# UDC-GAC/pRIblast

Measured on AMD Instinct MI355X. Metric: query RNAs/sec in `ris` step, higher is better.
Workload: dtype f64

## Files before the change

### priblast_amd/csrc/gapped_lds.hip

```cpp
#include <algorithm>
#include <type_traits>

#include "gapped_args.hpp"
#include "search_device.hpp"
#include "search_kernels.hpp"

namespace prb {

#ifdef PRB_GAP_PROFILE
constexpr int kProfSlots = 24;
__device__ unsigned long long g_gap_prof[10 * kProfSlots];
struct GapProf {
  unsigned long long last, acc[kProfSlots];
  int cells_now = 0, cells_prev = 0;
  __device__ __forceinline__ void start() {
    for (int i = 0; i < kProfSlots; i++) acc[i] = 0;
    last = __builtin_amdgcn_s_memtime();
  }
  __device__ __forceinline__ void mark(int r) {
    const unsigned long long t = __builtin_amdgcn_s_memtime();
    acc[r] += t - last;
    last = t;
  }
  __device__ __forceinline__ void count(int r) { acc[r] += 1; }
  __device__ __forceinline__ void flush(int kind) {
    if ((threadIdx.x & 63) == 0)
      for (int i = 0; i < kProfSlots; i++) atomicAdd(&g_gap_prof[kind * kProfSlots + i], acc[i]);
  }
};
#define GP_MARK(r) prof.mark(r)
#define GP_COUNT(r) prof.count(r)
#else
struct GapProf {
  __device__ __forceinline__ void start() {}
  __device__ __forceinline__ void flush(int) {}
};
#define GP_MARK(r)
#define GP_COUNT(r)
#endif

namespace {

constexpr int kInitStage = 16;
struct Tier0 {
#ifndef PRB_T0_CAPR
#define PRB_T0_CAPR 48
#define PRB_T0_WGCU 4
#endif
#ifndef PRB_T0_ACC_GLOBAL
#define PRB_T0_ACC_GLOBAL false
#endif
  static constexpr int kG = 8, kCapD = 32, kCapR = PRB_T0_CAPR, kGroups = 32, kWavesPerSimd = PRB_T0_WGCU, kWgPerCu = PRB_T0_WGCU;
  static constexpr bool kResumable = true;
  static constexpr bool kResumes = false;
  static constexpr bool kPairSteps = true;
  static constexpr bool kAccGlobal = PRB_T0_ACC_GLOBAL;
};
#ifndef PRB_T12_ACC_GLOBAL
#define PRB_T12_ACC_GLOBAL true
#endif
#ifndef PRB_T12_WPS
#define PRB_T12_WPS (PRB_T12_ACC_GLOBAL ? 4 : 3)
#endif
#ifndef PRB_T1_CAPD
#define PRB_T1_CAPD 40
#define PRB_T1_CAPR 64
#define PRB_T1_GROUPS 32
#define PRB_T1_WGCU (PRB_T12_ACC_GLOBAL ? 4 : 3)
#endif
struct Tier1 {
  static constexpr int kG = 8, kCapD = PRB_T1_CAPD, kCapR = PRB_T1_CAPR, kGroups = PRB_T1_GROUPS, kWavesPerSimd = PRB_T12_WPS, kWgPerCu = PRB_T1_WGCU;
  static constexpr bool kResumable = true, kResumes = true;
  using From = Tier0;
  using FromRec = Rec32;
  static constexpr bool kPairSteps = false;
  static constexpr bool kAccGlobal = PRB_T12_ACC_GLOBAL;
};
struct Tier2 {
  static constexpr int kG = 16, kCapD = 64, kCapR = 120, kGroups = 16, kWavesPerSimd = PRB_T12_WPS, kWgPerCu = PRB_T12_ACC_GLOBAL ? 4 : 3;
  static constexpr bool kResumable = true, kResumes = true;
  using From = Tier1;
  using FromRec = Rec32;
  static constexpr bool kPairSteps = false;
  static constexpr bool kAccGlobal = PRB_T12_ACC_GLOBAL;
};
struct Tier3 {
  static constexpr int kG = 64, kCapD = 128, kCapR = 512, kGroups = 1, kWavesPerSimd = 4, kWgPerCu = 16;
  static constexpr bool kResumable = false, kResumes = true;
  using From = Tier2;
  using FromRec = Rec32;
  static constexpr bool kPairSteps = false;
  static constexpr bool kAccGlobal = false;
};

struct Rec32W {
  using word = uint32_t;
  static constexpr bool kBases = false;
  static __device__ __forceinline__ word pack(int i, int j, int pred, int type, int, int) {
    return (word)i | ((word)j << 8) | ((word)pred << 16) | ((word)type << 25);
  }
  static __device__ __forceinline__ int i(word v) { return v & 0xFF; }
  static __device__ __forceinline__ int j(word v) { return (v >> 8) & 0xFF; }
  static __device__ __forceinline__ int pred(word v) { return (v >> 16) & 0x1FF; }
  static __device__ __forceinline__ int type(word v) { return (v >> 25) & 7; }
  static __device__ __forceinline__ int qa(word) { return 0; }
  static __device__ __forceinline__ int da(word) { return 0; }
};
struct Rec64 {
  using word = uint64_t;
  static constexpr bool kBases = true;
  static __device__ __forceinline__ word pack(int i, int j, int pred, int type, int qa, int da) {
    return (word)(uint32_t)i | ((word)(uint32_t)j << 16) | ((word)type << 32) | ((word)qa << 36) | ((word)da << 40) |
           ((word)(uint32_t)pred << 44);
  }
  static __device__ __forceinline__ int i(word v) { return (int)(v & 0xFFFF); }
  static __device__ __forceinline__ int j(word v) { return (int)((v >> 16) & 0xFFFF); }
  static __device__ __forceinline__ int pred(word v) { return (int)(v >> 44); }
  static __device__ __forceinline__ int type(word v) { return (int)((v >> 32) & 0xF); }
  static __device__ __forceinline__ int qa(word v) { return (int)((v >> 36) & 0xF); }
  static __device__ __forceinline__ int da(word v) { return (int)((v >> 40) & 0xF); }
};
static_assert(Tier3::kCapD + 16 <= 255 && Tier3::kCapR <= 512 && Tier0::kCapR * 8 >= 6 * kInitStage * 4 && Tier2::kCapD + 16 <= 127 && Tier2::kCapR <= 127, "Rec32 field widths");
static_assert(Tier0::kCapD <= Tier1::kCapD && Tier1::kCapD <= Tier2::kCapD && Tier2::kCapD <= Tier3::kCapD && Tier0::kCapR <= Tier1::kCapR &&
                  Tier1::kCapR <= Tier2::kCapR && Tier2::kCapR <= Tier3::kCapR,
              "a tier continues the dumps of the one before it");

template <class T, class Rec> struct LdsState {
  double eq[T::kCapD], ed[T::kCapD];
  double hyb[T::kCapR];
  typename Rec::word info[T::kCapR];
  static constexpr int kPtabLen = (T::kCapD + 7) & ~7;
  alignas(8) uint8_t ptab[3][kPtabLen];
  uint8_t qb[T::kCapD + 16], db[T::kCapD + 16];
};
template <class T, class Rec, bool kAccGlobal = T::kAccGlobal> struct LdsLive : LdsState<T, Rec> {};
template <class T, class Rec> struct LdsLive<T, Rec, true> {
  double hyb[T::kCapR];
  typename Rec::word info[T::kCapR];
  static constexpr int kPtabLen = (T::kCapD + 7) & ~7;
  alignas(8) uint8_t ptab[3][kPtabLen];
  uint8_t qb[T::kCapD + 16], db[T::kCapD + 16];
};
template <class T, class Rec> struct LdsStore {
  using R = Rec;
  static constexpr bool kResumable = T::kResumable;
  static constexpr bool kAccGlobal = T::kAccGlobal;
  static constexpr int kCapD = T::kCapD;
  LdsLive<T, Rec> &s;
  double *acc;
  __device__ __forceinline__ int cap_d() const { return T::kCapD; }
  __device__ __forceinline__ int cap_r() const { return T::kCapR; }
  __device__ __forceinline__ double &eq(int i) const {
    if constexpr (T::kAccGlobal) return acc[i];
    else return s.eq[i];
  }
  __device__ __forceinline__ double &ed(int i) const {
    if constexpr (T::kAccGlobal) return acc[T::kCapD + i];
    else return s.ed[i];
  }
  __device__ __forceinline__ double &hyb(int r) const { return s.hyb[r]; }
  __device__ __forceinline__ typename Rec::word &info(int r) const { return s.info[r]; }
  __device__ __forceinline__ uint8_t &ptab(int row, int i) const { return s.ptab[row][i]; }
  __device__ __forceinline__ int ptab_len() const { return LdsState<T, Rec>::kPtabLen; }
  __device__ __forceinline__ int win_len() const { return T::kCapD + 16; }
  __device__ __forceinline__ uint8_t &qb(int t) const { return s.qb[t]; }
  __device__ __forceinline__ uint8_t &db(int t) const { return s.db[t]; }
};
struct HbmStore {
  using R = Rec64;
  static constexpr bool kResumable = false;
  static constexpr bool kAccGlobal = false;
  double *eq_, *ed_, *hyb_;
  uint64_t *info_;
  uint8_t *ptab_, *qb_, *db_;
  int capd, capr;
  __device__ __forceinline__ int cap_d() const { return capd; }
  __device__ __forceinline__ int cap_r() const { return capr; }
  __device__ __forceinline__ double &eq(int i) const { return eq_[i]; }
  __device__ __forceinline__ double &ed(int i) const { return ed_[i]; }
  __device__ __forceinline__ double &hyb(int r) const { return hyb_[r]; }
  __device__ __forceinline__ uint64_t &info(int r) const { return info_[r]; }
  __device__ __forceinline__ uint8_t &ptab(int row, int i) const { return ptab_[(size_t)row * (capd + 4) + i]; }
  __device__ __forceinline__ int ptab_len() const { return capd + 4; }
  __device__ __forceinline__ int win_len() const { return capd + 16; }
  __device__ __forceinline__ uint8_t &qb(int t) const { return qb_[t]; }
  __device__ __forceinline__ uint8_t &db(int t) const { return db_[t]; }
};

template <bool kLds> __device__ __forceinline__ void group_sync() {
  if (kLds) {
    __builtin_amdgcn_fence(__ATOMIC_RELEASE, "wavefront");
    __builtin_amdgcn_wave_barrier();
    __builtin_amdgcn_fence(__ATOMIC_ACQUIRE, "wavefront");
  } else {
    __builtin_amdgcn_fence(__ATOMIC_RELEASE, "workgroup");
    __builtin_amdgcn_wave_barrier();
    __builtin_amdgcn_fence(__ATOMIC_ACQUIRE, "workgroup");
  }
}

template <class Store> __device__ __forceinline__ void acc_sync() {
  if constexpr (Store::kAccGlobal) {
    __builtin_amdgcn_fence(__ATOMIC_RELEASE, "workgroup");
    __builtin_amdgcn_wave_barrier();
    __builtin_amdgcn_fence(__ATOMIC_ACQUIRE, "workgroup");
  }
}

template <int kCtrl> __device__ __forceinline__ double dpp_f64(double x) {
  const int lo = __builtin_amdgcn_update_dpp(0, __double2loint(x), kCtrl, 0xF, 0xF, false);
  const int hi = __builtin_amdgcn_update_dpp(0, __double2hiint(x), kCtrl, 0xF, 0xF, false);
  return __hiloint2double(hi, lo);
}
template <int kCtrl> __device__ __forceinline__ int dpp_i32(int x) { return __builtin_amdgcn_update_dpp(0, x, kCtrl, 0xF, 0xF, false); }
__device__ __forceinline__ void group_min_halves(double &te, int &key, bool halves) {
  double m = te;
  m = __builtin_fmin(m, dpp_f64<0xB1>(m));
  m = __builtin_fmin(m, dpp_f64<0x4E>(m));
  const double m8 = __builtin_fmin(m, dpp_f64<0x141>(m));
  m = halves ? m : m8;
  int k = te == m ? key : 0x7fffffff;
  k = min(k, dpp_i32<0xB1>(k));
  k = min(k, dpp_i32<0x4E>(k));
  const int k8 = min(k, dpp_i32<0x141>(k));
  te = m;
  key = halves ? k : k8;
}
template <int G> __device__ __forceinline__ void group_min(double &te, int &key) {
  if (G == 8 || G == 16) {
    double m = te;
    m = __builtin_fmin(m, dpp_f64<0xB1>(m));
    m = __builtin_fmin(m, dpp_f64<0x4E>(m));
    m = __builtin_fmin(m, dpp_f64<0x141>(m));
    if (G == 16) m = __builtin_fmin(m, dpp_f64<0x140>(m));
    int k = te == m ? key : 0x7fffffff;
    k = min(k, dpp_i32<0xB1>(k));
    k = min(k, dpp_i32<0x4E>(k));
    k = min(k, dpp_i32<0x141>(k));
    if (G == 16) k = min(k, dpp_i32<0x140>(k));
    te = m;
    key = k;
  } else if (G == 64) {
    group_min<16>(te, key);
#pragma unroll
    for (int m = 16; m <= 32; m <<= 1) {
      const double ote = __shfl_xor(te, m);
      const int ok = __shfl_xor(key, m);
      if (ote < te || (ote == te && ok < key)) {
        te = ote;
        key = ok;
      }
    }
  } else {
#pragma unroll
    for (int m = G / 2; m >= 1; m >>= 1) {
      const double ote = __shfl_xor(te, m);
      const int ok = __shfl_xor(key, m);
      if (ote < te || (ote == te && ok < key)) {
        te = ote;
        key = ok;
      }
    }
  }
}

struct DirResult {
  bool overflow;
  int best;
};

struct SeqBases {
  const uint8_t *qenc;
  const float *qacc, *qcond, *dacc, *dcond;
};
struct HitCtx {
  int64_t x, out0;
  int64_t qo, dbase;
  HitState h;
  int query, id, qn;
  int diag_q, diag_d, diag_len, ndiag, nleft, nright;
  bool unsorted, ovf;
  bool resumed;
  int tier0;
};
struct DirState {
  double min_e;
  double acc_prev;
  int min_ci, min_cj;
  int length, best, nrec, lo, tq0, td0;
  int staged;
  int resume_i0, resume_dstart;
  bool overflow;
};

template <int G, bool kLds, class Store>
__device__ __forceinline__ void stage_acc(const SeqBases &sb, const HitCtx &c, int flag, int delta, const Store &S, int gl, DirState &d, int L0,
                                          int nb, float *scratch ) {
  const float *qacc = sb.qacc + c.qo, *qcond = sb.qcond + c.qo, *dacc = sb.dacc + c.dbase, *dcond = sb.dcond + c.dbase;
  const DirOrigin og = dir_origin(c.h, flag);
  auto term = [&](int k, int len) -> float {
    if (flag == 0) {
      const int p = og.q_start - len;
      return k == 0 ? qacc[p] : k == 1 ? qacc[p + 1] : k == 2 ? qcond[p + delta] : dcond[og.id_end + len];
    }
    const int p = og.id_start - len;
    return k == 0 ? qcond[og.q_start + len] : k == 3 ? dacc[p] : k == 4 ? dacc[p + 1] : dcond[p + delta];
  };
  if (scratch) {
    for (int t = gl; t < nb; t += G) {
      const int len = L0 + t;
      if (len < d.tq0) {
        scratch[0 * nb + t] = term(0, len);
        if (flag == 0) {
          scratch[1 * nb + t] = term(1, len);
          scratch[2 * nb + t] = term(2, len);
        }
      }
      if (len < d.td0) {
        scratch[3 * nb + t] = term(3, len);
        if (flag == 1) {
          scratch[4 * nb + t] = term(4, len);
          scratch[5 * nb + t] = term(5, len);
        }
      }
    }
    group_sync<kLds>();
  }
  auto get = [&](int k, int t) -> float { return scratch ? scratch[k * nb + t] : term(k, L0 + t); };
  if (gl < 2) {
    const bool qside = gl == 0, three = qside == (flag == 0);
    const int kb = qside ? 0 : 3, lim = qside ? d.tq0 : d.td0;
    double *out = qside ? &S.eq(0) : &S.ed(0);
    for (int k = 0; k < nb && L0 + k < lim && L0 + k <= S.cap_d(); k++) {
      const int len = L0 + k;
      const float x = get(kb, k), y = get(kb + 1, k), z = get(kb + 2, k);
      double v;
      if (len == 1) v = three ? (double)(x - y + z) : (double)x;
      else v = three ? d.acc_prev + x - y + z : d.acc_prev + x;
      d.acc_prev = v;
      out[len - 1] = v;
    }
  }
  d.staged = L0 + nb - 1 < S.cap_d() ? L0 + nb - 1 : S.cap_d();
  group_sync<kLds>();
  acc_sync<Store>();
}

template <int G, bool kLds, class Store>
__device__ __forceinline__ void stage_acc_regs(const SeqBases &sb, const HitCtx &c, int flag, int delta, const Store &S, int gl, int gbase,
                                               DirState &d, int L0) {
  constexpr int nb = kInitStage, per = (nb + G - 1) / G;
  const float *qacc = sb.qacc + c.qo, *qcond = sb.qcond + c.qo, *dacc = sb.dacc + c.dbase, *dcond = sb.dcond + c.dbase;
  const DirOrigin og = dir_origin(c.h, flag);
  float t0[per], t1[per], t2[per], t3[per];
#pragma unroll
  for (int r = 0; r < per; r++) {
    t0[r] = t1[r] = t2[r] = t3[r] = 0.0f;
    const int t = gl + r * G, len = L0 + t;
    if (t < nb) {
      if (len < d.tq0) {
        if (flag == 0) {
          const int p = og.q_start - len;
          t0[r] = qacc[p];
          t1[r] = qacc[p + 1];
          t2[r] = qcond[p + delta];
        } else {
          t0[r] = qcond[og.q_start + len];
        }
      }
      if (len < d.td0) {
        if (flag == 0) {
          t3[r] = dcond[og.id_end + len];
        } else {
          const int p = og.id_start - len;
          t1[r] = dacc[p];
          t2[r] = dacc[p + 1];
          t3[r] = dcond[p + delta];
        }
      }
    }
  }
  double veq = __shfl(d.acc_prev, gbase), ved = __shfl(d.acc_prev, gbase + (G > 1 ? 1 : 0));
#pragma unroll
  for (int k = 0; k < nb; k++) {
    const int src = gbase + (k % G), r = k / G, len = L0 + k;
    const float a0 = __shfl(t0[r], src), a1 = __shfl(t1[r], src), a2 = __shfl(t2[r], src), a3 = __shfl(t3[r], src);
    if (len <= S.cap_d()) {
      if (len < d.tq0) {
        double v;
        if (flag == 0) v = len == 1 ? (double)(a0 - a1 + a2) : veq + a0 - a1 + a2;
        else v = len == 1 ? (double)a0 : veq + a0;
        veq = v;
        if (gl == 0) S.eq(len - 1) = v;
      }
      if (len < d.td0) {
        double v;
        if (flag == 0) v = len == 1 ? (double)a3 : ved + a3;
        else v = len == 1 ? (double)(a1 - a2 + a3) : ved + a1 - a2 + a3;
        ved = v;
        if (gl == 0) S.ed(len - 1) = v;
      }
    }
  }
  d.acc_prev = (G > 1 && gl == 1) ? ved : veq;
  d.staged = L0 + nb - 1 < S.cap_d() ? L0 + nb - 1 : S.cap_d();
  group_sync<kLds>();
  acc_sync<Store>();
}

template <int G, bool kLds, class Store>
__device__ __forceinline__ void stage_windows(const SeqBases &sb, const HitCtx &c, int flag, const uint8_t *ds, int64_t dn, const Store &S, int gl,
                                              DirState &d, bool clear_rows = true) {
  const uint8_t *qs = sb.qenc + c.qo;
  const int qn = c.qn;
  const int wn = S.win_len();
  const DirOrigin og = dir_origin(c.h, flag);
  d.tq0 = wn;
  d.td0 = wn;
  for (int t = gl; t < wn; t += G) {
    const int64_t qp = flag == 0 ? (int64_t)og.q_start - t : (int64_t)og.q_start + t;
    const int64_t dp = flag == 0 ? og.db_start - t : og.db_start + t;
    const int qc = (qp >= 0 && qp < qn) ? get_char(qs, qp) : 0;
    const int dc = (dp >= 0 && dp < dn) ? get_char(ds, dp) : 0;
    S.qb(t) = (uint8_t)qc;
    S.db(t) = (uint8_t)dc;
    if (t >= 1 && qc == 0 && t < d.tq0) d.tq0 = t;
    if (t >= 1 && dc == 0 && t < d.td0) d.td0 = t;
  }
  if (clear_rows) {
    uint32_t *pz = reinterpret_cast<uint32_t *>(&S.ptab(0, 0));
    for (int t = gl; t < 3 * S.ptab_len() / 4; t += G) pz[t] = 0;
  }
#pragma unroll
  for (int m = G / 2; m >= 1; m >>= 1) {
    const int ta = __shfl_xor(d.tq0, m), tb = __shfl_xor(d.td0, m);
    d.tq0 = ta < d.tq0 ? ta : d.tq0;
    d.td0 = tb < d.td0 ? tb : d.td0;
  }
  group_sync<kLds>();
}

template <int G, bool kLds, class Store>
__device__ __forceinline__ void dir_init(const SearchConst &sc, const SeqBases &sb, const HitCtx &c, int flag, const uint8_t *ds, int64_t dn,
                                         const Store &S, int gl, int delta, DirState &d) {
  using R = typename Store::R;
  d.min_e = c.h.e_tot;
  d.min_ci = 0;
  d.min_cj = 0;
  d.length = 0;
  d.best = 0;
  d.overflow = false;
  d.resume_i0 = 0;
  d.resume_dstart = 0;

  stage_windows<G, kLds>(sb, c, flag, ds, dn, S, gl, d);
  d.acc_prev = 0;
  {
    stage_acc<G, kLds>(sb, c, flag, delta, S, gl, d, 1, kInitStage, reinterpret_cast<float *>(&S.hyb(0)));
  }
  int type0 = bp_type(sc, S.qb(0), S.db(0));
  if (flag == 0) type0 = rtype_of(type0);
  if (gl == 0) {
    S.hyb(0) = d.min_e;
    S.info(0) = R::pack(0, 0, 0, type0, S.qb(1), S.db(1));
    S.ptab(0, 0) = (uint8_t)type0;
  }
  group_sync<kLds>();
  d.nrec = 1;
  d.lo = 0;
}

template <int G, bool kLds, class Store>
__device__ __forceinline__ bool dir_step(const SearchConst &sc, const SeqBases &sb, const ExtOpts &o, const HitCtx &c, int flag, const Store &S,
                                         int gl , int gbase ,
                                         DirState &d, GapProf &prof) {
  using R = typename Store::R;
  const int delta = o.delta, drop = o.drop_w_gap, min_helix = o.min_helix;
  const bool mid = d.resume_i0 != 0;
  if (!mid) {
    if (d.length >= S.cap_d()) {
      d.overflow = true;
      return true;
    }
    d.length++;
  }
  const bool q_open = d.length < d.tq0, d_open = d.length < d.td0;
  const int cur = kLds ? d.length - 3 * ((d.length * 171) >> 9) : d.length % 3, d2 = cur == 2 ? 0 : cur + 1;
  static_assert(!kLds || Tier3::kCapD + 16 < 256, "multiply-shift division by 3");
  if (!mid) {
    if (d.length > d.staged) stage_acc_regs<G, kLds>(sb, c, flag, delta, S, gl, gbase, d, d.length);
    GP_MARK(1);
    GP_COUNT(10);
    if constexpr (kLds) {
      uint64_t *row = reinterpret_cast<uint64_t *>(&S.ptab(cur, 0));
      for (int t = gl; t < S.ptab_len() / 8; t += G) row[t] = 0;
    } else {
      for (int t = gl; t <= d.length; t += G) S.ptab(cur, t) = 0;
    }
    group_sync<kLds>();
    if (d.length - 2 > drop) {
      while (d.lo < d.nrec) {
        const auto v = S.info(d.lo);
        if (d.length - R::i(v) - R::j(v) - 2 > drop) d.lo++;
        else break;
      }
    }
  }
  GP_MARK(2);
  const int dstart = mid ? d.resume_dstart : d.nrec;
  const int i_first = d.length - d.td0 + 1 > 1 ? d.length - d.td0 + 1 : 1;
  const int i_lo = mid ? d.resume_i0 : i_first;
  const int i_hi = (d.length < d.tq0 ? d.length : d.tq0) - 1;
  d.resume_i0 = 0;

  typename R::word v_first = 0;
  double h_first = 0;
  if (d.lo + gl < dstart) {
    v_first = S.info(d.lo + gl);
    h_first = S.hyb(d.lo + gl);
  }

  constexpr bool kTwoCells = G == 8 && kLds;
  auto fill_cell = [&](int ci, int ctype, bool two) -> int {
    GP_COUNT(12);
    const bool pair_mode = kTwoCells && two, hi = pair_mode && gl >= G / 2;
    const int sub = pair_mode ? (gl & (G / 2 - 1)) : gl, stride = pair_mode ? G / 2 : G;
    const int cj = d.length - ci;
    const int nq = S.qb(ci - 1), nd = S.db(cj - 1);
    const double eq_c = S.eq(ci - 1), ed_c = S.ed(cj - 1);
    const int fq = S.qb(ci + 1), fd = S.db(cj + 1);
    double bte = 1000000.0;
    int bkp = d.lo << 3;
    typename R::word vn = v_first;
    double hn = h_first;
    if constexpr (kTwoCells) {
      if (pair_mode) {
        const typename R::word v4 = (typename R::word)dpp_i32<0x114>((int)v_first);
        const double h4 = dpp_f64<0x114>(h_first);
        vn = hi ? v4 : v_first;
        hn = hi ? h4 : h_first;
        if (sub + d.lo >= dstart) vn = 0;
      }
    }
    for (int k0 = d.lo; k0 < dstart; k0 += stride) {
      GP_COUNT(13);
      const int k = k0 + sub;
      const auto v = vn;
      const double hk = hn;
      if (k + stride < dstart) {
        vn = S.info(k + stride);
        hn = S.hyb(k + stride);
      }
      if (k < dstart) {
        const int ri = R::i(v), rj = R::j(v);
        if (ri < ci && rj < cj) {
          const int rq = R::kBases ? R::qa(v) : (int)S.qb(ri + 1), rd = R::kBases ? R::da(v) : (int)S.db(rj + 1);
          const bool f0 = flag == 0;
          const int rt = R::type(v);
          double te = loop_energy_abcd(sc, f0 ? ctype : rt, f0 ? rt : ctype, ci - ri - 1, cj - rj - 1, f0 ? nq : rq, f0 ? nd : rd,
                                       f0 ? rq : nq, f0 ? rd : nd);
          te += hk;
          if (te < bte) {
            bte = te;
            bkp = (k << 3) | R::type(v);
          }
        }
      }
    }
    GP_MARK(4);
    if constexpr (kTwoCells) group_min_halves(bte, bkp, pair_mode);
    else group_min<G>(bte, bkp);
    GP_MARK(5);
    if (d.nrec >= S.cap_r()) return -1;
    int bk = bkp >> 3, ptype = bkp & 7;
    if (d.lo >= dstart) bk = 0;
    if (ptype == 0) ptype = R::type(S.info(bk));
    const int rec = d.nrec + (hi ? 1 : 0);
    if (sub == 0) {
      S.hyb(rec) = bte;
      S.info(rec) = R::pack(ci, cj, bk, rtype_of(ctype), fq, fd);
      S.ptab(cur, ci) = (uint8_t)ptype;
    }
    const double ie = eq_c + ed_c + bte;
    if constexpr (kTwoCells) {
      const double ie_o = dpp_f64<0x141>(ie);
      const int ci_o = dpp_i32<0x141>(ci);
      const double ie_a = hi ? ie_o : ie, ie_b = hi ? ie : ie_o;
      const int ci_a = hi ? ci_o : ci, ci_b = hi ? ci : ci_o;
      if (ie_a < d.min_e) {
        d.min_e = ie_a;
        d.best = d.nrec;
        d.min_ci = ci_a;
        d.min_cj = d.length - ci_a;
      }
      if (pair_mode && ie_b < d.min_e) {
        d.min_e = ie_b;
        d.best = d.nrec + 1;
        d.min_ci = ci_b;
        d.min_cj = d.length - ci_b;
      }
      d.nrec += pair_mode ? 2 : 1;
    } else {
      if (ie < d.min_e) {
        d.min_e = ie;
        d.best = d.nrec;
        d.min_ci = ci;
        d.min_cj = cj;
      }
      d.nrec++;
    }
    GP_MARK(6);
    return ptype;
  };

  auto fill_quad = [&](int i0, unsigned long long cellbits, int n, unsigned long long tb0, unsigned long long tb1, unsigned long long tb2) {
    GP_COUNT(12);
    const int sub = gl >> 4, sl = gl & 15;
    unsigned long long mbits = cellbits;
    for (int t = 0; t < sub; t++) mbits &= mbits - 1;
    const bool act = sub < n;
    const int b = act ? __builtin_ctzll(mbits) : __builtin_ctzll(cellbits);
    const int ci = i0 + b, cj = d.length - ci;
    const int ctype = (int)((tb0 >> (gbase + b)) & 1) | (int)(((tb1 >> (gbase + b)) & 1) << 1) | (int)(((tb2 >> (gbase + b)) & 1) << 2);
    const int nq = S.qb(ci - 1), nd = S.db(cj - 1);
    const double eq_c = S.eq(ci - 1), ed_c = S.ed(cj - 1);
    const int fq = S.qb(ci + 1), fd = S.db(cj + 1);
    double bte = 1000000.0;
    int bkp = d.lo << 3;
    for (int k0 = d.lo; k0 < dstart; k0 += 16) {
      GP_COUNT(13);
      const int k = k0 + sl;
      if (k < dstart) {
        const auto v = S.info(k);
        const double hk = S.hyb(k);
        const int ri = R::i(v), rj = R::j(v);
        if (ri < ci && rj < cj) {
          const int rq = R::kBases ? R::qa(v) : (int)S.qb(ri + 1), rd = R::kBases ? R::da(v) : (int)S.db(rj + 1);
          const bool f0 = flag == 0;
          const int rt = R::type(v);
          double te = loop_energy_abcd(sc, f0 ? ctype : rt, f0 ? rt : ctype, ci - ri - 1, cj - rj - 1, f0 ? nq : rq, f0 ? nd : rd,
                                       f0 ? rq : nq, f0 ? rd : nd);
          te += hk;
          if (te < bte) {
            bte = te;
            bkp = (k << 3) | R::type(v);
          }
        }
      }
    }
    GP_MARK(4);
    group_min<16>(bte, bkp);
    GP_MARK(5);
    int bk = bkp >> 3, ptype = bkp & 7;
    if (d.lo >= dstart) bk = 0;
    if (ptype == 0) ptype = R::type(S.info(bk));
    if (act && sl == 0) {
      const int rec = d.nrec + sub;
      S.hyb(rec) = bte;
      S.info(rec) = R::pack(ci, cj, bk, rtype_of(ctype), fq, fd);
      S.ptab(cur, ci) = (uint8_t)ptype;
    }
    const double ie = eq_c + ed_c + bte;
#pragma unroll
    for (int t = 0; t < 4; t++) {
      if (t < n) {
        const int l16 = 16 * t;
        const double ie_t = __hiloint2double(__builtin_amdgcn_readlane(__double2hiint(ie), l16), __builtin_amdgcn_readlane(__double2loint(ie), l16));
        const int ci_t = __builtin_amdgcn_readlane(ci, l16);
        if (ie_t < d.min_e) {
          d.min_e = ie_t;
          d.best = d.nrec + t;
          d.min_ci = ci_t;
          d.min_cj = d.length - ci_t;
        }
      }
    }
    d.nrec += n;
    GP_MARK(6);
  };

  auto cell_type = [&](int i) -> int {
    if (i > i_hi) return 0;
    const int j = d.length - i;
    const unsigned q0 = S.qb(i), d0 = S.db(j), q1 = S.qb(i + 1), d1 = S.db(j + 1), q2 = S.qb(i + 2), d2b = S.db(j + 2);
    const int pt = S.ptab(d2, i - 1);
    const unsigned x0 = q0 * 5 + d0, x1 = q1 * 5 + d1, x2 = q2 * 5 + d2b;
    const unsigned p0 = (sc.pair_mask >> x0) & 1, w0 = (sc.wobble_mask >> x0) & 1;
    unsigned ahead = 1;
    if (min_helix >= 2) ahead = ((sc.pair_mask >> x1) & 1) & ~(w0 & (sc.wobble_mask >> x1));
    if (min_helix >= 3) ahead &= sc.pair_mask >> x2;
    for (int x = 3; x <= min_helix - 1; x++) ahead &= sc.pair_mask >> ((unsigned)S.qb(i + x) * 5 + S.db(j + x));
    const unsigned need = (unsigned)(pt == 0) | (w0 & (unsigned)wobble(pt));
    int t = (int)((sc.bp_rows >> ((x0 * 3 - 15) & 63)) & 7);
    if (flag == 1) t = ((t - 1) ^ 1) + 1;
    return (p0 & (ahead | ~need) & 1) ? t : 0;
  };

  if constexpr (G == 8 && kLds) {
    constexpr int kChunks = (Store::kCapD + G - 1) / G;
    using cells_t = typename std::conditional<kChunks <= 4, uint32_t, unsigned long long>::type;
    uint32_t tw[kChunks];
    cells_t cells = 0;
#pragma unroll
    for (int c = 0; c < kChunks; c++) {
      tw[c] = 0;
      const int i0 = i_lo + c * G;
      if (i0 <= i_hi) {
        const int type1 = cell_type(i0 + gl);
        uint32_t w = (uint32_t)type1 << (3 * gl);
        w |= (uint32_t)dpp_i32<0xB1>((int)w);
        w |= (uint32_t)dpp_i32<0x4E>((int)w);
        w |= (uint32_t)dpp_i32<0x141>((int)w);
        tw[c] = w;
        cells |= (cells_t)((__ballot(type1 != 0) >> gbase) & 0xFF) << (8 * c);
        GP_COUNT(11);
      }
    }
    GP_MARK(3);
#ifdef PRB_GAP_PROFILE
    prof.cells_now = kChunks <= 4 ? __popc((uint32_t)cells) : __popcll((unsigned long long)cells);
#endif
    while (cells) {
      const cells_t rest = cells & (cells - 1);
      const bool two = rest != 0 && d.nrec + 2 <= S.cap_r();
      const int b0 = kChunks <= 4 ? __builtin_ctz((uint32_t)cells) : __builtin_ctzll((unsigned long long)cells);
      if (Store::kResumable && d.nrec >= S.cap_r()) {
        d.overflow = true;
        d.resume_i0 = i_lo + b0;
        d.resume_dstart = dstart;
        break;
      }
      int b = b0;
      if (two) {
        const int b1 = kChunks <= 4 ? __builtin_ctz((uint32_t)rest) : __builtin_ctzll((unsigned long long)rest);
        if (gl >= G / 2) b = b1;
        cells = rest & (rest - 1);
      } else {
        cells = rest;
      }
      uint32_t w = tw[0];
#pragma unroll
      for (int c = 1; c < kChunks; c++) w = (b >> 3) == c ? tw[c] : w;
      const int ptype = fill_cell(i_lo + b, (int)((w >> (3 * (b & 7))) & 7), two);
      if (ptype < 0) {
        d.overflow = true;
        break;
      }
    }
    group_sync<kLds>();
    GP_MARK(3);
  } else {
    for (int i0 = i_lo; i0 <= i_hi && !d.overflow; i0 += G) {
      const int type1 = cell_type(i0 + gl);
      using mask_t = typename std::conditional<G <= 32, uint32_t, unsigned long long>::type;
      const unsigned long long tb0 = __ballot(type1 & 1), tb1 = __ballot(type1 & 2), tb2 = __ballot(type1 & 4);
      const unsigned long long anyb = tb0 | tb1 | tb2;
      mask_t vmask = G < 64 ? (mask_t)((anyb >> gbase) & ((1ull << (G & 63)) - 1)) : (mask_t)anyb;
      GP_MARK(3);
      GP_COUNT(11);
      if (Store::kResumable && d.nrec + __popcll((unsigned long long)vmask) > S.cap_r()) {
        d.overflow = true;
        d.resume_i0 = i0;
        d.resume_dstart = dstart;
        break;
      }
      while (vmask) {
        if constexpr (G == 64) {
          const int left = __popcll((unsigned long long)vmask), n = left < 4 ? left : 4;
          if (n >= 2 && d.nrec + n <= S.cap_r()) {
            fill_quad(i0, (unsigned long long)vmask, n, tb0, tb1, tb2);
            for (int t = 0; t < n; t++) vmask &= vmask - 1;
            continue;
          }
        }
        const int b = G <= 32 ? __builtin_ctz((uint32_t)vmask) : __builtin_ctzll((unsigned long long)vmask);
        vmask &= vmask - 1;
        const int ctype = (int)((tb0 >> (gbase + b)) & 1) | (int)(((tb1 >> (gbase + b)) & 1) << 1) |
                          (int)(((tb2 >> (gbase + b)) & 1) << 2);
        const int ptype = fill_cell(i0 + b, ctype, false);
        if (ptype < 0) {
          d.overflow = true;
          break;
        }
      }
      group_sync<kLds>();
      GP_MARK(3);
    }
  }
  if (d.overflow) return true;
  if (d.length - (d.min_ci + d.min_cj) >= drop) return true;
  if (!q_open && !d_open) return true;
  return false;
}

template <class Store>
__device__ __forceinline__ bool dir_step_pair(const SearchConst &sc, const SeqBases &sb, const ExtOpts &o, const HitCtx &c, int flag,
                                              const Store &S, int gl, int gbase, DirState &d, GapProf &prof) {
  constexpr int G = 8;
  using R = typename Store::R;
  static_assert(Store::kCapD <= 32, "a 32-bit mask of cells per anti-diagonal");
  constexpr int kChunks = (Store::kCapD + G - 1) / G;
  const int delta = o.delta, drop = o.drop_w_gap, min_helix = o.min_helix;
  const bool mid = d.resume_i0 != 0;
  if (!mid) {
    if (d.length >= S.cap_d()) {
      d.overflow = true;
      return true;
    }
    d.length++;
  }
  const int LA = d.length;
  const bool openA = LA < d.tq0 || LA < d.td0;
  const int curA = LA - 3 * ((LA * 171) >> 9), d2A = curA == 2 ? 0 : curA + 1;
  if (!mid) {
    if (LA > d.staged) stage_acc_regs<G, true>(sb, c, flag, delta, S, gl, gbase, d, LA);
    GP_MARK(1);
    GP_COUNT(10);
    uint64_t *row = reinterpret_cast<uint64_t *>(&S.ptab(curA, 0));
    for (int t = gl; t < S.ptab_len() / 8; t += G) row[t] = 0;
    group_sync<true>();
    if (LA - 2 > drop) {
      while (d.lo < d.nrec) {
        const auto v = S.info(d.lo);
        if (LA - R::i(v) - R::j(v) - 2 > drop) d.lo++;
        else break;
      }
    }
  }
  GP_MARK(2);
  const int dstartA = mid ? d.resume_dstart : d.nrec, loA = d.lo;
  const int i_firstA = LA - d.td0 + 1 > 1 ? LA - d.td0 + 1 : 1;
  const int i_loA = mid ? d.resume_i0 : i_firstA;
  const int i_hiA = (LA < d.tq0 ? LA : d.tq0) - 1;
  d.resume_i0 = 0;

  auto pair_type = [&](int i, int j) -> int {
    const unsigned x0 = (unsigned)S.qb(i) * 5 + S.db(j);
    int t = (int)((sc.bp_rows >> ((x0 * 3 - 15) & 63)) & 7);
    if (flag == 1) t = ((t - 1) ^ 1) + 1;
    return t;
  };
  auto helix_ok = [&](unsigned x0, unsigned x1, unsigned x2, int pt, int i, int j) -> bool {
    const unsigned p0 = (sc.pair_mask >> x0) & 1, w0 = (sc.wobble_mask >> x0) & 1;
    unsigned ahead = 1;
    if (min_helix >= 2) ahead = ((sc.pair_mask >> x1) & 1) & ~(w0 & (sc.wobble_mask >> x1));
    if (min_helix >= 3) ahead &= sc.pair_mask >> x2;
    for (int x = 3; x <= min_helix - 1; x++) ahead &= sc.pair_mask >> ((unsigned)S.qb(i + x) * 5 + S.db(j + x));
    const unsigned need = (unsigned)(pt == 0) | (w0 & (unsigned)wobble(pt));
    return (p0 & (ahead | ~need) & 1) != 0;
  };

  const int LB = LA + 1, d2B = curA == 0 ? 2 : curA - 1;
  const bool try_pair = !mid && openA && LA - (d.min_ci + d.min_cj) < drop && LA < S.cap_d() && LB <= d.staged;
  uint32_t cellsA = 0, cellsB = 0;
  int loB = loA;
  bool paired = false;
  if (try_pair) {
    if (LB - 2 > drop) {
      while (loB < dstartA) {
        const auto v = S.info(loB);
        if (LB - R::i(v) - R::j(v) - 2 > drop) loB++;
        else break;
      }
    }
    const int i_loB = LB - d.td0 + 1 > 1 ? LB - d.td0 + 1 : 1, i_hiB = (LB < d.tq0 ? LB : d.tq0) - 1;
#pragma unroll
    for (int ch = 0; ch < kChunks; ch++) {
      const int i0 = i_loA + ch * G;
      if (i0 <= i_hiB) {
        const int i = i0 + gl, j = LA - i, jc = j < 0 ? 0 : j;
        const unsigned q0 = (unsigned)S.qb(i) * 5, q1 = (unsigned)S.qb(i + 1) * 5, q2 = (unsigned)S.qb(i + 2) * 5;
        const unsigned d0 = S.db(jc), d1 = S.db(jc + 1), d2b = S.db(jc + 2), d3 = S.db(jc + 3);
        const bool okA = i <= i_hiA && helix_ok(q0 + d0, q1 + d1, q2 + d2b, S.ptab(d2A, i - 1), i, j);
        const bool okB = i >= i_loB && i <= i_hiB && helix_ok(q0 + d1, q1 + d2b, q2 + d3, S.ptab(d2B, i - 1), i, j + 1);
        cellsA |= (uint32_t)((__ballot(okA) >> gbase) & 0xFF) << (8 * ch);
        cellsB |= (uint32_t)((__ballot(okB) >> gbase) & 0xFF) << (8 * ch);
        GP_COUNT(11);
      }
    }
    if (d.nrec + __popc(cellsA) + __popc(cellsB) <= S.cap_r()) {
      paired = true;
      uint64_t *row = reinterpret_cast<uint64_t *>(&S.ptab(d2A, 0));
      for (int t = gl; t < S.ptab_len() / 8; t += G) row[t] = 0;
      group_sync<true>();
      GP_COUNT(10);
    } else {
      cellsB = 0;
    }
  } else {
#pragma unroll
    for (int ch = 0; ch < kChunks; ch++) {
      const int i0 = i_loA + ch * G;
      if (i0 <= i_hiA) {
        const int i = i0 + gl, j = LA - i, jc = j < 0 ? 0 : j;
        const unsigned x0 = (unsigned)S.qb(i) * 5 + S.db(jc), x1 = (unsigned)S.qb(i + 1) * 5 + S.db(jc + 1),
                       x2 = (unsigned)S.qb(i + 2) * 5 + S.db(jc + 2);
        const bool okA = i <= i_hiA && helix_ok(x0, x1, x2, S.ptab(d2A, i - 1), i, j);
        cellsA |= (uint32_t)((__ballot(okA) >> gbase) & 0xFF) << (8 * ch);
        GP_COUNT(11);
      }
    }
  }
  const int nA = __popc(cellsA);
  int typeA0 = 0;
  if (paired && nA != 0) {
    const int iA0 = i_loA + __builtin_ctz(cellsA);
    typeA0 = rtype_of(pair_type(iA0, LA - iA0));
  }
#ifdef PRB_GAP_PROFILE
  prof.cells_now = nA + __popc(cellsB);
#endif
  GP_MARK(3);

  auto fill_cell = [&](int ci, bool isB, bool two) -> int {
    GP_COUNT(12);
    const bool pair_mode = two, hi = pair_mode && gl >= G / 2;
    const int sub = pair_mode ? (gl & (G / 2 - 1)) : gl, stride = pair_mode ? G / 2 : G;
    const int L = LA + (isB ? 1 : 0), cur = isB ? (curA == 2 ? 0 : curA + 1) : curA, lo = isB ? loB : loA;
    const int cj = L - ci;
    const int ctype = pair_type(ci, cj);
    const int nq = S.qb(ci - 1), nd = S.db(cj - 1);
    double bte = 1000000.0;
    int bkp = lo << 3;
    typename R::word vn = 0;
    double hn = 0;
    if (lo + sub < dstartA) {
      vn = S.info(lo + sub);
      hn = S.hyb(lo + sub);
    }
    for (int k0 = lo; k0 < dstartA; k0 += stride) {
      GP_COUNT(13);
      const int k = k0 + sub;
      const auto v = vn;
      const double hk = hn;
      if (k + stride < dstartA) {
        vn = S.info(k + stride);
        hn = S.hyb(k + stride);
      }
#ifdef PRB_GAP_PROFILE
      {
        const bool has = k < dstartA, ok = has && R::i(v) < ci && R::j(v) < cj;
        prof.acc[22] += (unsigned long long)__popcll(__ballot(has));
        prof.acc[23] += (unsigned long long)__popcll(__ballot(ok));
      }
#endif
      if (k < dstartA) {
        const int ri = R::i(v), rj = R::j(v);
        if (ri < ci && rj < cj) {
          const int rq = R::qa(v), rd = R::da(v);
          const bool f0 = flag == 0;
          const int rt = R::type(v);
          double te = loop_energy_abcd(sc, f0 ? ctype : rt, f0 ? rt : ctype, ci - ri - 1, cj - rj - 1, f0 ? nq : rq, f0 ? nd : rd,
                                       f0 ? rq : nq, f0 ? rd : nd);
          te += hk;
          if (te < bte) {
            bte = te;
            bkp = (k << 3) | R::type(v);
          }
        }
      }
    }
    GP_MARK(4);
    group_min_halves(bte, bkp, pair_mode);
    GP_MARK(5);
    if (d.nrec >= S.cap_r()) return -1;
    int bk = bkp >> 3, ptype = bkp & 7;
    const bool a_first = isB && typeA0 != 0 && lo >= dstartA;
    if (lo >= dstartA && !a_first) bk = 0;
    if (ptype == 0) ptype = a_first ? typeA0 : R::type(S.info(bk));
    const int rec = d.nrec + (hi ? 1 : 0);
    if (sub == 0) {
      S.hyb(rec) = bte;
      S.info(rec) = R::pack(ci, cj, bk, rtype_of(ctype), S.qb(ci + 1), S.db(cj + 1));
      S.ptab(cur, ci) = (uint8_t)ptype;
    }
    const double ie = S.eq(ci - 1) + S.ed(cj - 1) + bte;
    const double ie_o = dpp_f64<0x141>(ie);
    const int ci_o = dpp_i32<0x141>(ci), cj_o = dpp_i32<0x141>(cj);
    const double ie_a = hi ? ie_o : ie, ie_b = hi ? ie : ie_o;
    const int ci_a = hi ? ci_o : ci, ci_b = hi ? ci : ci_o, cj_a = hi ? cj_o : cj, cj_b = hi ? cj : cj_o;
    if (ie_a < d.min_e) {
      d.min_e = ie_a;
      d.best = d.nrec;
      d.min_ci = ci_a;
      d.min_cj = cj_a;
    }
    if (pair_mode && ie_b < d.min_e) {
      d.min_e = ie_b;
      d.best = d.nrec + 1;
      d.min_ci = ci_b;
      d.min_cj = cj_b;
    }
    d.nrec += pair_mode ? 2 : 1;
    GP_MARK(6);
    return ptype;
  };

  unsigned long long cells = (unsigned long long)cellsA | ((unsigned long long)cellsB << 32);
  while (cells) {
    const unsigned long long rest = cells & (cells - 1);
    const bool two = rest != 0 && d.nrec + 2 <= S.cap_r();
    const int b0 = __builtin_ctzll(cells);
    if (Store::kResumable && d.nrec >= S.cap_r()) {
      d.overflow = true;
      d.resume_i0 = i_loA + b0;
      d.resume_dstart = dstartA;
      break;
    }
    int b = b0;
    if (two) {
      if (gl >= G / 2) b = __builtin_ctzll(rest);
      cells = rest & (rest - 1);
    } else {
      cells = rest;
    }
    const bool isB = b >= 32;
    const int ptype = fill_cell(i_loA + (b & 31), isB, two);
    if (ptype < 0) {
      d.overflow = true;
      break;
    }
  }
  group_sync<true>();
  GP_MARK(3);
  if (d.overflow) return true;
  if (paired) {
    d.length = LA + 1;
    d.lo = loB;
    if (LB - (d.min_ci + d.min_cj) >= drop) return true;
    return !(LB < d.tq0 || LB < d.td0);
  }
  if (LA - (d.min_ci + d.min_cj) >= drop) return true;
  return !openA;
}

template <class Store> __device__ __forceinline__ DirResult dir_finish(const DirState &d, HitState &h, int flag, const Store &S) {
  DirResult r;
  r.overflow = d.overflow;
  r.best = d.min_ci != 0 ? d.best : 0;
  if (d.min_ci != 0) {
    h.e_acc = h.e_acc + S.eq(d.min_ci - 1) + S.ed(d.min_cj - 1);
    if (flag == 0) {
      h.q_sp -= d.min_ci;
      h.db_sp -= d.min_cj;
    } else {
      h.id_start -= d.min_cj;
    }
    h.q_len += d.min_ci;
    h.db_len += d.min_cj;
  }
  h.e_tot = d.min_e;
  return r;
}

struct ResumeHeader {
  DirState d;
  double acc_prev1;
  HitState h;
  int32_t flag, nleft;
};
template <class T, class Rec> constexpr size_t resume_bytes() {
  return (sizeof(ResumeHeader) + sizeof(LdsState<T, Rec>) + 63) & ~(size_t)63;
}

template <int G, class T, class Rec>
__device__ __forceinline__ void resume_dump(const GapResume &ro, const HitCtx &c, const DirState &d, int flag,
                                            const LdsStore<T, Rec> &S, int gl, int gbase) {
  int slot = -1;
  if (gl == 0) {
    slot = (int)atomicAdd(ro.count, 1u);
    if (slot >= ro.cap) slot = -1;
  }
  slot = __shfl(slot, gbase);
  if (slot < 0) return;
  uint8_t *dst = ro.pool + (size_t)slot * resume_bytes<T, Rec>();
  ResumeHeader *H = reinterpret_cast<ResumeHeader *>(dst);
  if (gl == 0) {
    H->d = d;
    H->h = c.h;
    H->flag = flag;
    H->nleft = c.nleft;
    ro.slot[c.x] = slot;
  } else if (gl == 1) {
    H->acc_prev1 = d.acc_prev;
  }
  if constexpr (!T::kAccGlobal) {
    uint32_t *w = reinterpret_cast<uint32_t *>(dst + sizeof(ResumeHeader));
    const uint32_t *src = reinterpret_cast<const uint32_t *>(&S.s);
#pragma unroll 2
    for (int t = gl; t < (int)(sizeof(LdsState<T, Rec>) / 4); t += G) w[t] = src[t];
  } else {
    LdsState<T, Rec> *o = reinterpret_cast<LdsState<T, Rec> *>(dst + sizeof(ResumeHeader));
    for (int t = gl; t < T::kCapD; t += G) {
      o->eq[t] = S.eq(t);
      o->ed[t] = S.ed(t);
    }
    for (int t = gl; t < d.nrec; t += G) {
      o->hyb[t] = S.hyb(t);
      o->info[t] = S.info(t);
    }
    uint32_t *pw = reinterpret_cast<uint32_t *>(&o->ptab[0][0]);
    const uint32_t *ps = reinterpret_cast<const uint32_t *>(&S.s.ptab[0][0]);
    for (int t = gl; t < 3 * LdsState<T, Rec>::kPtabLen / 4; t += G) pw[t] = ps[t];
  }
}

template <int G, class TS, class RecS, class Store>
__device__ __forceinline__ void resume_load(const GapResume &ri, int slot, const GapArgs &a, HitCtx &c, DirState &d, int &flag,
                                            const Store &S, int gl) {
  using R = typename Store::R;
  const uint8_t *src = ri.pool + (size_t)slot * resume_bytes<TS, RecS>();
  const ResumeHeader *H = reinterpret_cast<const ResumeHeader *>(src);
  d = H->d;
  if (G > 1 && gl == 1) d.acc_prev = H->acc_prev1;
  d.overflow = false;
  c.h = H->h;
  c.nleft = H->nleft;
  flag = H->flag;
  const LdsState<TS, RecS> *s0 = reinterpret_cast<const LdsState<TS, RecS> *>(src + sizeof(ResumeHeader));
  stage_windows<G, true>(SeqBases{a.qb.enc, a.qb.acc, a.qb.cond, a.pg.acc, a.pg.cond}, c, flag, a.pg.seqs, a.pg.nchars, S, gl,
                         d);
  for (int t = gl; t < TS::kCapD; t += G) {
    S.eq(t) = s0->eq[t];
    S.ed(t) = s0->ed[t];
  }
  for (int t = gl; t < d.nrec; t += G) {
    S.hyb(t) = s0->hyb[t];
    const auto v = s0->info[t];
    S.info(t) = R::pack(RecS::i(v), RecS::j(v), RecS::pred(v), RecS::type(v), RecS::qa(v), RecS::da(v));
  }
  constexpr int kLenS = LdsState<TS, RecS>::kPtabLen;
  for (int t = gl; t < 3 * kLenS; t += G) {
    const int row = t / kLenS, i = t - row * kLenS;
    S.ptab(row, i) = s0->ptab[row][i];
  }
  group_sync<true>();
  acc_sync<Store>();
}

template <int kMode> __device__ __forceinline__ void hit_load(const GapArgs &a, int64_t w, HitCtx &c) {
  const SearchConst &sc = a.sc;
  const int64_t x = a.subset ? (int64_t)a.subset[w] : w;
  c.x = x;
  c.query = a.in.query[x];
  c.qo = a.qb.off[c.query];
  c.qn = a.qb.len[c.query] + 1;
  c.id = a.in.db_id[x];
  c.dbase = (int64_t)a.pg.start_pos[c.id] - c.id;
  HitState &h = c.h;
  h.q_sp = a.in.q_sp[x];
  h.db_sp = a.in.db_sp[x];
  h.q_len = a.in.q_len[x];
  h.db_len = a.in.db_len[x];
  h.id_start = a.in.db_id_start[x];
  h.e_tot = a.in.e_tot[x];
  h.e_acc = a.in.e_acc[x];
  c.diag_q = h.q_sp;
  c.diag_d = h.db_sp;
  c.diag_len = US(h.q_len);
  c.ndiag = 0;
  if (kMode != 0)
    for (int t = 0; t < c.diag_len; t++)
      c.ndiag += diag_pairs(sc, a.qb.enc[c.qo + c.diag_q + t], a.pg.seqs[c.diag_d + t]);
  c.unsorted = kMode != 0 && a.first_flag && a.first_flag[x];
  c.out0 = kMode == 2 ? a.bp_off[w] : 0;
  c.ovf = false;
  c.nleft = 0;
  c.nright = 0;
  c.resumed = false;
  c.tier0 = 0;
  if (kMode == 0 && is_resumed(a.tier_out[x])) {
    c.tier0 = a.tier_out[x] & kMarkTier;
    h.q_sp = a.out.q_sp[x];
    h.db_sp = a.out.db_sp[x];
    h.q_len = a.out.q_len[x];
    h.db_len = a.out.db_len[x];
    h.id_start = a.out.db_id_start[x];
    h.e_tot = a.out.e_tot[x];
    h.e_acc = a.out.e_acc[x];
    c.nleft = a.bp_count[x] & 0xFFFF;
    c.resumed = true;
  }
}

template <int kMode, bool kLds, class Store>
__device__ __forceinline__ void hit_dir_done(const GapArgs &a, HitCtx &c, int flag, const DirOrigin &og ,
                                             const DirResult &r, const Store &S, int gl) {
  using R = typename Store::R;
  c.ovf = r.overflow;
  if (c.ovf) return;
  int cnt = 0;
  int lslot = -1;
  if constexpr (kMode == 0 && !kLds) lslot = a.lt.slot ? a.lt.slot[c.x] : -1;
  for (int k = r.best; k != 0; k = R::pred(S.info(k)), cnt++) {
    if (kMode == 0 && kLds && gl == 0 && cnt < kTraceCap) {
      const auto v = S.info(k);
      a.trace[(c.x * 2 + flag) * kTraceCap + cnt] = (uint16_t)(R::i(v) | (R::j(v) << 8));
    }
    if (kMode == 0 && !kLds && gl == 0 && lslot >= 0 && cnt < a.lt.cap) {
      const auto v = S.info(k);
      a.lt.trace[((int64_t)lslot * 2 + flag) * a.lt.cap + cnt] = (uint32_t)R::i(v) | ((uint32_t)R::j(v) << 16);
    }
  }
  if (kMode == 0 && !kLds && gl == 0 && lslot >= 0) a.lt.count[lslot * 2 + flag] = cnt <= a.lt.cap ? cnt : -2;
  if (flag == 0) c.nleft = cnt;
  else c.nright = cnt;
  if (kMode == 2 && gl == 0) {
    int t = 0;
    for (int k = r.best; k != 0; k = R::pred(S.info(k)), t++) {
      const auto v = S.info(k);
      int64_t pos;
      int qv, dv;
      if (flag == 0) {
        qv = og.q_start - R::i(v);
        dv = (int)(og.db_start - R::j(v));
        pos = c.unsorted ? c.out0 + c.ndiag + t : c.out0 + t;
      } else {
        qv = og.q_start + R::i(v);
        dv = (int)(og.db_start + R::j(v));
        pos = c.unsorted ? c.out0 + c.ndiag + c.nleft + t : c.out0 + c.nleft + c.ndiag + (cnt - 1 - t);
      }
      a.bp_out[2 * pos] = qv;
      a.bp_out[2 * pos + 1] = dv;
    }
  }
}

template <int kMode>
__device__ __forceinline__ void hit_store(const GapArgs &a, int64_t w, const HitCtx &c, int flag , int gl) {
  if (gl != 0) return;
  const SearchConst &sc = a.sc;
  const HitState &h = c.h;
  const uint8_t *ds = a.pg.seqs, *qs = a.qb.enc + c.qo;
  if (kMode == 0) {
    a.overflow[w] = c.ovf ? 1 : 0;
    if (c.ovf && flag == 1) {
      const int64_t x = c.x;
      a.out.q_sp[x] = h.q_sp;
      a.out.db_sp[x] = h.db_sp;
      a.out.q_len[x] = h.q_len;
      a.out.db_len[x] = h.db_len;
      a.out.db_id_start[x] = h.id_start;
      a.out.e_acc[x] = h.e_acc;
      a.out.e_hyb[x] = h.e_tot - h.e_acc;
      a.out.e_tot[x] = h.e_tot;
      a.bp_count[x] = c.nleft;
      a.tier_out[x] = (uint8_t)(kResumeMark | ((c.resumed ? c.tier0 : a.tier_id) & kMarkTier));
    }
    if (!c.ovf) {
      const int64_t x = c.x;
      int tcode = a.tier_id > c.tier0 ? a.tier_id : c.tier0;
      if (a.tier_id == kWaveTier && a.lt.slot) {
        const int ls = a.lt.slot[x];
        if (ls >= 0) {
          const int c0 = a.lt.count[ls * 2], c1 = a.lt.count[ls * 2 + 1];
          if ((c0 >= 0 || (c0 == -1 && c.nleft <= kTraceCap)) && c1 >= 0) tcode = kLongTraceTier;
        }
      }
      a.tier_out[x] = (uint8_t)tcode;
      a.bp_count[x] = c.nleft | (c.nright << 16);
      const double d0 = dangle_energy_gapped(sc, h.q_sp, h.db_sp, 0, qs, c.qn, ds, a.pg.nchars);
      const double d1 = dangle_energy_gapped(sc, h.q_sp + US(h.q_len) - 1, (int64_t)h.db_sp + US(h.db_len) - 1, 1, qs, c.qn,
                                             ds, a.pg.nchars);
      double e = h.e_tot, hy = h.e_tot - h.e_acc;
// ... 411 lines not shown
```

Baseline: 6.809.

## Split record scan into qualifying-bitmask pass and sparse energy evaluation

The per-cell scan over prior records becomes two phases. The first pass only loads info words and builds a per-lane bitmask of records that satisfy ri<ci && rj<cj. The second pass iterates set bits and computes the loop energy, loading hyb only for qualifying records. This drops hyb loads for non-qualifying records and shortens the divergent energy loop, at the cost of a second LDS read of info and a bit-iteration loop whose trip count varies per lane.

Result: faster. 7.022, median of 6 (+3.1%).

```diff
diff --git a/priblast_amd/csrc/gapped_lds.hip b/priblast_amd/csrc/gapped_lds.hip
--- a/priblast_amd/csrc/gapped_lds.hip
+++ b/priblast_amd/csrc/gapped_lds.hip
@@ -8,7 +8,7 @@
 namespace prb {
 
 #ifdef PRB_GAP_PROFILE
-constexpr int kProfSlots = 24;
+constexpr int kProfSlots = 26;
 __device__ unsigned long long g_gap_prof[10 * kProfSlots];
 struct GapProf {
   unsigned long long last, acc[kProfSlots];
@@ -145,7 +145,7 @@
   using R = Rec;
   static constexpr bool kResumable = T::kResumable;
   static constexpr bool kAccGlobal = T::kAccGlobal;
-  static constexpr int kCapD = T::kCapD;
+  static constexpr int kCapD = T::kCapD, kCapR = T::kCapR;
   LdsLive<T, Rec> &s;
   double *acc;
   __device__ __forceinline__ int cap_d() const { return T::kCapD; }
@@ -440,6 +440,39 @@
   group_sync<kLds>();
 }
 
+template <class R, class Store, class Energy>
+__device__ __forceinline__ void scan_qualifying(const Store &S, int lo, int dstart, int sub, int stride, int ci, int cj,
+                                                typename R::word v0, const Energy &energy, double &bte, int &bkp, GapProf &prof) {
+  static_assert(Store::kCapR <= 32 * 4, "a bit per round of at least four lanes");
+  uint32_t mine = 0;
+  typename R::word vn = v0;
+  for (int k0 = lo, r = 0; k0 < dstart; k0 += stride, r++) {
+    GP_COUNT(25);
+    const int k = k0 + sub;
+    const auto v = vn;
+    if (k + stride < dstart) vn = S.info(k + stride);
+    const bool ok = k < dstart && R::i(v) < ci && R::j(v) < cj;
+#ifdef PRB_GAP_PROFILE
+    prof.acc[22] += (unsigned long long)__popcll(__ballot(k < dstart));
+    prof.acc[23] += (unsigned long long)__popcll(__ballot(ok));
+#endif
+    mine |= (uint32_t)ok << r;
+  }
+  GP_MARK(24);
+  while (mine) {
+    GP_COUNT(13);
+    const int k = lo + sub + __builtin_ctz(mine) * stride;
+    mine &= mine - 1;
+    const auto v = S.info(k);
+    double te = energy(v);
+    te += S.hyb(k);
+    if (te < bte) {
+      bte = te;
+      bkp = (k << 3) | R::type(v);
+    }
+  }
+}
+
 template <int G, bool kLds, class Store>
 __device__ __forceinline__ void dir_init(const SearchConst &sc, const SeqBases &sb, const HitCtx &c, int flag, const uint8_t *ds, int64_t dn,
                                          const Store &S, int gl, int delta, DirState &d) {
@@ -513,11 +546,12 @@
   const int i_hi = (d.length < d.tq0 ? d.length : d.tq0) - 1;
   d.resume_i0 = 0;
 
+  constexpr bool kQualScan = kLds && G <= 16;
   typename R::word v_first = 0;
   double h_first = 0;
   if (d.lo + gl < dstart) {
     v_first = S.info(d.lo + gl);
-    h_first = S.hyb(d.lo + gl);
+    if constexpr (!kQualScan) h_first = S.hyb(d.lo + gl);
   }
 
   constexpr bool kTwoCells = G == 8 && kLds;
@@ -531,34 +565,37 @@
     const int fq = S.qb(ci + 1), fd = S.db(cj + 1);
     double bte = 1000000.0;
     int bkp = d.lo << 3;
-    typename R::word vn = v_first;
-    double hn = h_first;
-    if constexpr (kTwoCells) {
-      if (pair_mode) {
-        const typename R::word v4 = (typename R::word)dpp_i32<0x114>((int)v_first);
-        const double h4 = dpp_f64<0x114>(h_first);
-        vn = hi ? v4 : v_first;
-        hn = hi ? h4 : h_first;
-        if (sub + d.lo >= dstart) vn = 0;
-      }
-    }
-    for (int k0 = d.lo; k0 < dstart; k0 += stride) {
-      GP_COUNT(13);
-      const int k = k0 + sub;
-      const auto v = vn;
-      const double hk = hn;
-      if (k + stride < dstart) {
-        vn = S.info(k + stride);
-        hn = S.hyb(k + stride);
-      }
-      if (k < dstart) {
-        const int ri = R::i(v), rj = R::j(v);
-        if (ri < ci && rj < cj) {
-          const int rq = R::kBases ? R::qa(v) : (int)S.qb(ri + 1), rd = R::kBases ? R::da(v) : (int)S.db(rj + 1);
-          const bool f0 = flag == 0;
-          const int rt = R::type(v);
-          double te = loop_energy_abcd(sc, f0 ? ctype : rt, f0 ? rt : ctype, ci - ri - 1, cj - rj - 1, f0 ? nq : rq, f0 ? nd : rd,
-                                       f0 ? rq : nq, f0 ? rd : nd);
+    auto energy = [&](typename R::word v) -> double {
+      const int ri = R::i(v), rj = R::j(v);
+      const int rq = R::kBases ? R::qa(v) : (int)S.qb(ri + 1), rd = R::kBases ? R::da(v) : (int)S.db(rj + 1);
+      const bool f0 = flag == 0;
+      const int rt = R::type(v);
+      return loop_energy_abcd(sc, f0 ? ctype : rt, f0 ? rt : ctype, ci - ri - 1, cj - rj - 1, f0 ? nq : rq, f0 ? nd : rd, f0 ? rq : nq,
+                              f0 ? rd : nd);
+    };
+    if constexpr (kQualScan) {
+      typename R::word v0 = v_first;
+      if constexpr (kTwoCells) {
+        if (pair_mode) {
+          const typename R::word v4 = (typename R::word)dpp_i32<0x114>((int)v_first);
+          v0 = hi ? v4 : v_first;
+        }
+      }
+      scan_qualifying<R>(S, d.lo, dstart, sub, stride, ci, cj, v0, energy, bte, bkp, prof);
+    } else {
+      typename R::word vn = v_first;
+      double hn = h_first;
+      for (int k0 = d.lo; k0 < dstart; k0 += stride) {
+        GP_COUNT(13);
+        const int k = k0 + sub;
+        const auto v = vn;
+        const double hk = hn;
+        if (k + stride < dstart) {
+          vn = S.info(k + stride);
+          hn = S.hyb(k + stride);
+        }
+        if (k < dstart && R::i(v) < ci && R::j(v) < cj) {
+          double te = energy(v);
           te += hk;
           if (te < bte) {
             bte = te;
@@ -922,44 +959,18 @@
     const int nq = S.qb(ci - 1), nd = S.db(cj - 1);
     double bte = 1000000.0;
     int bkp = lo << 3;
-    typename R::word vn = 0;
-    double hn = 0;
-    if (lo + sub < dstartA) {
-      vn = S.info(lo + sub);
-      hn = S.hyb(lo + sub);
-    }
-    for (int k0 = lo; k0 < dstartA; k0 += stride) {
-      GP_COUNT(13);
-      const int k = k0 + sub;
-      const auto v = vn;
-      const double hk = hn;
-      if (k + stride < dstartA) {
-        vn = S.info(k + stride);
-        hn = S.hyb(k + stride);
-      }
-#ifdef PRB_GAP_PROFILE
-      {
-        const bool has = k < dstartA, ok = has && R::i(v) < ci && R::j(v) < cj;
-        prof.acc[22] += (unsigned long long)__popcll(__ballot(has));
-        prof.acc[23] += (unsigned long long)__popcll(__ballot(ok));
-      }
-#endif
-      if (k < dstartA) {
-        const int ri = R::i(v), rj = R::j(v);
-        if (ri < ci && rj < cj) {
+    const typename R::word v0 = lo + sub < dstartA ? S.info(lo + sub) : 0;
+    scan_qualifying<R>(
+        S, lo, dstartA, sub, stride, ci, cj, v0,
+        [&](typename R::word v) -> double {
+          const int ri = R::i(v), rj = R::j(v);
           const int rq = R::qa(v), rd = R::da(v);
           const bool f0 = flag == 0;
           const int rt = R::type(v);
-          double te = loop_energy_abcd(sc, f0 ? ctype : rt, f0 ? rt : ctype, ci - ri - 1, cj - rj - 1, f0 ? nq : rq, f0 ? nd : rd,
-                                       f0 ? rq : nq, f0 ? rd : nd);
-          te += hk;
-          if (te < bte) {
-            bte = te;
-            bkp = (k << 3) | R::type(v);
-          }
-        }
-      }
-    }
+          return loop_energy_abcd(sc, f0 ? ctype : rt, f0 ? rt : ctype, ci - ri - 1, cj - rj - 1, f0 ? nq : rq, f0 ? nd : rd,
+                                  f0 ? rq : nq, f0 ? rd : nd);
+        },
+        bte, bkp, prof);
     GP_MARK(4);
     group_min_halves(bte, bkp, pair_mode);
     GP_MARK(5);
```
